# HandH1998/QQQ

Hardware: AMD Instinct MI355X
Metric: W4A8 GEMM TOPS + speedup vs fp16, M in {1..4096} N=8192 K=21760 (higher is better)
Workload: dtype i8 x i4 -> i32 -> f16; 1 GPU; qqq_gemm per-channel sweep M in {1,16,128,1024,4096} N=8192 K=21760 (configs[1]); step = the 5 calls; weights=12 rotating 89 MB int4 buffers (cold Infinity Cache), GPTQ-style N(0,0.02^2), launch=hipGraph replay, 1-step opener then 10 steps/graph, parallelism=single GPU

## Files before the change

qqq_amd/csrc/qqq_wide.hip.h:

```cpp
#ifndef QQQ_AMD_QQQ_WIDE_HIP_H_
#define QQQ_AMD_QQQ_WIDE_HIP_H_


#ifndef QQQ_WIDE_ABLATE
#define QQQ_WIDE_ABLATE 0
#endif
#ifdef QQQ_PANEL_TRACE
#define QQQ_WTRV(i, v)                                                                                   \
  do {                                                                                                   \
    if (wn == 0 && qqq_trace_buf) qqq_trace_buf[(size_t)blockIdx.x * 16 + (i)] = (unsigned long long)(v); \
  } while (0)
#define QQQ_WTR(i) QQQ_WTRV(i, wall_clock64())
#else
#define QQQ_WTR(i) do {} while (0)
#define QQQ_WTRV(i, v) do {} while (0)
#endif
template <int... S, class F>
__device__ __forceinline__ void qqq_static_for(std::integer_sequence<int, S...>, F&& f) {
  (f(std::integral_constant<int, S>{}), ...);
}
template <int N, class F>
__device__ __forceinline__ void qqq_static_for(F&& f) {
  qqq_static_for(std::make_integer_sequence<int, N>{}, static_cast<F&&>(f));
}

__device__ __forceinline__ __amdgpu_buffer_rsrc_t wide_view(const void* base_uniform) {
  return __builtin_amdgcn_make_buffer_rsrc(const_cast<void*>(base_uniform), 0, 0xffffffff, 0x00020000);
}
__device__ __forceinline__ v4u wide_load16(__amdgpu_buffer_rsrc_t view, const unsigned voff, const unsigned soff) {
  return __builtin_amdgcn_raw_buffer_load_b128(view, voff, soff, 0);
}

__host__ __device__ constexpr bool wide_frag_slot(int hw, int k) { return k % (2 * hw) == 2 * hw - 1; }
__host__ __device__ constexpr int wide_dw_load_index(int mt, int hw, int k) {
  if (hw == 2) {
    if (mt == 8) {
      constexpr int at[8] = {2, 5, 6, 10, 14, 18, 22, 26};
      for (int i = 0; i < 8; ++i)
        if (at[i] == k) return i;
      return -1;
    }
    return (k % 4 == 2 && k <= 30) ? (k - 2) / 4 : -1;
  }
  return k == 2 ? 0 : k == 8 ? 1 : k == 10 ? 2 : k == 16 ? 3 : -1;
}
__host__ __device__ constexpr int wide_ring_load(int mode, int mt, int hw, int k) {
  if (mode == 2) return k % ((2 * hw * mt) / (2 * hw)) == 2 ? k / ((2 * hw * mt) / (2 * hw)) : -1;
  return wide_dw_load_index(mt, hw, k);
}
__host__ __device__ constexpr int wide_ring_last_slot(int mt, int hw, int hf) {
  int last = 0;
  for (int k = 0; k < 2 * hw * mt; ++k)
    if (wide_dw_load_index(mt, hw, k) == 4 * hf + 3) last = k;
  return last;
}
__host__ __device__ constexpr int wide_dma_period(int mt, int hw) { return (2 * hw * mt) / (mt / 4); }
__host__ __device__ constexpr bool wide_m0_slot(int mt, int hw, int k) { return k % wide_dma_period(mt, hw) == (hw == 2 ? 8 : 4); }
__host__ __device__ constexpr bool wide_dma_slot(int mt, int hw, int k) { return k % wide_dma_period(mt, hw) == (hw == 2 ? 9 : 6); }
__host__ __device__ constexpr int wide_scale_slot(int hw) { return hw == 2 ? 1 : 0; }

__host__ __device__ constexpr int wide_w8_refill_index_(int mt, int hw, int k) { return k % ((2 * hw * mt) / (2 * hw)) == 2 ? k / ((2 * hw * mt) / (2 * hw)) : -1; }
__host__ __device__ constexpr bool wide_plain_slot(int mode, int mt, int hw, int k) {
  if (k < 0 || k >= 2 * hw * mt) return false;
  if (wide_frag_slot(hw, k) || wide_dma_slot(mt, hw, k) || wide_m0_slot(mt, hw, k)) return false;
  if (wide_ring_load(mode, mt, hw, k) >= 0) return false;
  if (mode == 1 && k == wide_scale_slot(hw)) return false;
  return true;
}
__host__ __device__ constexpr int wide_barrier_slot(int mode, int mt, int hw) {
  for (int k = 2 * hw * mt - 1; k >= 0; --k)
    if (wide_plain_slot(mode, mt, hw, k)) return k;
  return 0;
}
__host__ __device__ constexpr int wide_plain_after(int mode, int mt, int hw, int k0, int skip) {
  int last = -1;
  for (int k = k0 + 1; k < 2 * hw * mt; ++k)
    if (wide_plain_slot(mode, mt, hw, k) && k != wide_barrier_slot(mode, mt, hw)) {
      last = k;
      if (skip-- == 0) return k;
    }
  return last;
}
__host__ __device__ constexpr int wide_ring_inc_slot(int mode, int mt, int hw) {
  int last = 0;
  for (int k = 0; k < 2 * hw * mt; ++k)
    if (wide_ring_load(mode, mt, hw, k) >= 0) last = k;
  return wide_plain_after(mode, mt, hw, last, 1);
}
__host__ __device__ constexpr int wide_dma_inc_slot(int, int, int) { return 0; }
__host__ __device__ constexpr int wide_scale_inc_slot(int mode, int mt, int hw) { return wide_plain_after(mode, mt, hw, wide_scale_slot(hw), 2); }
__host__ __device__ constexpr int wide_bal_cap(int mode, int mt, int hw, int t, int k, int cursors) {
  if (!wide_plain_slot(mode, mt, hw, k)) return wide_m0_slot(mt, hw, k) && !wide_frag_slot(hw, k) && !wide_dma_slot(mt, hw, k) ? 1 : 0;
  int c = 2;
  if (t == 1 && k == wide_barrier_slot(mode, mt, hw)) c -= 2;
  if (cursors == 1) {
    if (k == wide_ring_inc_slot(mode, mt, hw)) c -= 1;
    if (t == 0 && k == wide_dma_inc_slot(mode, mt, hw)) c -= 1;
    if (mode == 1 && t == 1 && k == wide_scale_inc_slot(mode, mt, hw)) c -= 1;
  }
  return c < 0 ? 0 : c;
}
__host__ __device__ constexpr int wide_bal_items(int mode) { return 1 + (mode == 1 ? 32 : 12); }
__host__ __device__ constexpr int wide_bal_cost(int mode, int w) { return w == 0 ? 1 : (mode == 1 ? 2 : 1); }
__host__ __device__ constexpr int wide_bal_before(int mode, int mt, int hw, int t, int k, int cursors) {
  const int nslot = 2 * hw * mt, per = wide_bal_items(mode), ni = hw * per;
  int ct = 0, cb = 0, tc = 0;
  for (int j = 0; j < nslot; ++j) ct += wide_bal_cap(mode, mt, hw, t, j, cursors);
  for (int j = 0; j < k; ++j) cb += wide_bal_cap(mode, mt, hw, t, j, cursors);
  for (int i = 0; i < ni; ++i) tc += wide_bal_cost(mode, i % per);
  if (k >= nslot) return ni;
  int n = 0, e = 0;
  for (int i = 0; i < ni; ++i) {
    e += wide_bal_cost(mode, i % per);
    if ((long long)e * ct <= (long long)cb * tc) ++n;
  }
  return n;
}

template <int MODE, int MT, int HW, int T, int CURSORS>
struct WideBalTable {
  struct Tab {
    int before[2 * HW * MT + 1];
  };
  static constexpr Tab make() {
    Tab r{};
    constexpr int nslot = 2 * HW * MT, per = wide_bal_items(MODE), ni = HW * per;
    int cap[nslot] = {};
    int ct = 0, tc = 0;
    for (int j = 0; j < nslot; ++j) {
      cap[j] = wide_bal_cap(MODE, MT, HW, T, j, CURSORS);
      ct += cap[j];
    }
    for (int i = 0; i < ni; ++i) tc += wide_bal_cost(MODE, i % per);
    int cb = 0, n = 0, e = wide_bal_cost(MODE, 0);
    for (int k = 0; k < nslot; ++k) {
      while (n < ni && (long long)e * ct <= (long long)cb * tc) {
        ++n;
        if (n < ni) e += wide_bal_cost(MODE, n % per);
      }
      r.before[k] = n;
      cb += cap[k];
    }
    r.before[nslot] = ni;
    return r;
  }
  static constexpr Tab tab = make();
};

static_assert(WideBalTable<0, 16, 2, 0, 1>::tab.before[17] == wide_bal_before(0, 16, 2, 0, 17, 1) && WideBalTable<0, 16, 2, 1, 1>::tab.before[63] == wide_bal_before(0, 16, 2, 1, 63, 1) &&
                  WideBalTable<1, 8, 2, 1, 0>::tab.before[9] == wide_bal_before(1, 8, 2, 1, 9, 0) && WideBalTable<1, 16, 1, 0, 0>::tab.before[30] == wide_bal_before(1, 16, 1, 0, 30, 0),
              "the table is the function");

__host__ __device__ constexpr int wide_w8_refill_index(int mt, int hw, int k) {
  const int per = (2 * hw * mt) / (2 * hw);
  return k % per == 2 ? k / per : -1;
}
__host__ __device__ constexpr int wide_loads_in_slot(int mode, int mt, int hw, int t, int k) {
  int n = 0;
  if (mode == 1 && t == 1 && k == wide_scale_slot(hw) && !(QQQ_WIDE_ABLATE & 8)) n += 2;
  if (mode != 2 && wide_ring_load(mode, mt, hw, k) >= 0 && !(QQQ_WIDE_ABLATE & 8)) n += 1;
  if (mode == 2 && wide_w8_refill_index(mt, hw, k) >= 0 && !(QQQ_WIDE_ABLATE & 8)) n += 1;
  if (wide_dma_slot(mt, hw, k) && !(QQQ_WIDE_ABLATE & 2)) n += 1;
  return n;
}
__host__ __device__ constexpr int wide_loads_in_step(int mode, int mt, int hw, int t, int from, int to) {
  int n = 0;
  for (int k = from; k < to && k < 2 * hw * mt; ++k) n += wide_loads_in_slot(mode, mt, hw, t, k);
  return n;
}
__host__ __device__ constexpr int wide_loads_between(int mode, int mt, int hw, int t0, int k0, int steps, int k1) {
  int n = wide_loads_in_step(mode, mt, hw, t0, k0 + 1, 2 * hw * mt);
  for (int j = 1; j < steps; ++j) n += wide_loads_in_step(mode, mt, hw, (t0 + j) & 1, 0, 2 * hw * mt);
  return n + wide_loads_in_step(mode, mt, hw, (t0 + steps) & 1, 0, k1);
}
__host__ __device__ constexpr int wide_w8_last_refill_slot(int mt, int hw) {
  int last = 0;
  for (int k = 0; k < 2 * hw * mt; ++k) last = wide_w8_refill_index(mt, hw, k) >= 0 ? k : last;
  return last;
}
__host__ __device__ constexpr int wide_last_dma_slot(int mt, int hw) {
  int last = 0;
  for (int k = 0; k < 2 * hw * mt; ++k) last = wide_dma_slot(mt, hw, k) ? k : last;
  return last;
}

template <int MODE, int MT, int P, int RS, int HW, bool CHAIN = false>
__global__ __launch_bounds__(256) __attribute__((amdgpu_waves_per_eu(1, 1))) void qqq_wide_kernel(
    const int8_t* __restrict__ A, const unsigned char* __restrict__ B, int32_t* __restrict__ C, _Float16* __restrict__ D,
    const float* __restrict__ s1, const float* __restrict__ s2, const _Float16* __restrict__ s3,
    int32_t* __restrict__ acc_out, int* __restrict__ tickets, const _Float16* __restrict__ bias, const int M, const int N,
    const int K, const int tiles_m, const int tiles_n, const int PW, const int ksplit_hf) {
  const int ksplit = ksplit_hf & 0xffff, hflags = (ksplit_hf >> 16) & 0xff, skew = (ksplit_hf >> 24) & 0x3f;
  constexpr bool GROUPED = MODE == 1, W8 = MODE == 2;
  static_assert(MODE >= 0 && MODE <= 2, "0 per-channel, 1 per-group, 2 expanded int8");
  static_assert(!W8 || RS >= 3, "W8: a slot is refilled one step after its use -- RS - 1 steps of lead, the wait count needs at least one whole step in between");
  constexpr int RL = W8 ? RS - 1 : RS;
  static_assert(MT == 16 || MT == 8, "m-tiles of 16 tokens per wave (= per workgroup): 256 or 128 tokens");
  static_assert(HW == 2 || HW == 1, "a wave owns both 32-column halves of a 64-column group, or (128-column tiles) one");
  constexpr int ROWS = 16 * MT;
  constexpr int NQ = 2 * HW;
  constexpr int BN = 128 * HW;
  constexpr int NT = 256;
  constexpr int XB = ROWS * 128;
  constexpr int XPT = XB / 16 / NT;
  static_assert((2 * P) % RS == 0, "weight ring (in 64-k steps) must divide the unroll period");
  static_assert(P >= 4 && P <= 6, "LDS stage buffers: one being read, one complete, P - 2 in flight");
  constexpr int LA = P - 1;
  constexpr int NSLOT = NQ * MT;
  constexpr int EPR = HW == 2 ? 8 * MT : 16 * MT;
  constexpr int EP_STRIDE = BN + 4;

  extern __shared__ __attribute__((aligned(16))) unsigned char smem[];

  const int tid = threadIdx.x;
  const int lane = tid & 63;
  const int wn = __builtin_amdgcn_readfirstlane(tid >> 6);
  QQQ_WTR(0);

  int tile_m, tile_n, tile_lin, sp;
  auto locate = [&](const int lin, int& tm, int& tn) {
    const int full = (tiles_n / PW) * PW * tiles_m;
    if (lin < full) {
      const int panel = lin / (PW * tiles_m), within = lin % (PW * tiles_m);
      tm = within / PW;
      tn = panel * PW + within % PW;
    } else {
      const int rem = lin - full, pw = tiles_n % PW;
      tm = rem / pw;
      tn = (tiles_n / PW) * PW + rem % pw;
    }
  };
  int ch_first = 0, ch_stride = 0, ch_tiles = 1;
  {
    const int ntot = tiles_m * tiles_n * (CHAIN ? 1 : ksplit);
    const int bid = blockIdx.x;
    const int q = ntot >> 3, rr = ntot & 7;
    const int xcd = bid & 7, idx = bid >> 3;
    const int lin2 = (xcd < rr ? xcd * (q + 1) : rr * (q + 1) + (xcd - rr) * q) + idx;
    if constexpr (CHAIN) {
      const int cnt = q + (xcd < rr ? 1 : 0);
      ch_stride = (int)(gridDim.x >> 3);
      ch_first = lin2;
      ch_tiles = idx < cnt ? (cnt - idx + ch_stride - 1) / ch_stride : 0;
      if (ch_tiles == 0) return;
      sp = 0;
      tile_lin = lin2;
      locate(lin2, tile_m, tile_n);
    } else if (ksplit == 2 && (hflags & 16) != 0 && ((tiles_m * tiles_n) & 3) == 0) {
      const int per = (tiles_m * tiles_n) >> 2;
      sp = xcd & 1;
      tile_lin = (xcd >> 1) * per + idx;
      locate(tile_lin, tile_m, tile_n);
    } else {
      const int lin = lin2 / ksplit;
      sp = lin2 - lin * ksplit;
      tile_lin = lin;
      locate(lin, tile_m, tile_n);
    }
  }
  unsigned my_xcc = 0;
  if (!CHAIN && ksplit > 1) {
    asm volatile("s_getreg_b32 %0, hwreg(HW_REG_XCC_ID)" : "=s"(my_xcc));
    my_xcc &= 7u;
    if (tid == 0 && ksplit <= 6)
      __hip_atomic_fetch_or(tickets + 2 * (size_t)tile_lin, (int)((8u | my_xcc) << (8 + 4 * sp)), __ATOMIC_RELAXED, __HIP_MEMORY_SCOPE_AGENT);
  }
  const int mbase = tile_m * ROWS;
  const int ngroups = N >> 6;
  const int cb = tile_n * 4 + wn;
  int ng = HW == 2 ? cb : cb >> 1;
  const int whalf = HW == 2 ? 0 : (cb & 1);
  if (ng >= ngroups) ng = ngroups - 1;
  const unsigned rowbytes = (unsigned)N * 8u;
  const unsigned wstep = W8 ? (unsigned)N * 64u : 4u * rowbytes;

  const int NSE = (K >> 7) - skew;
  const int st0 = (int)(((long long)NSE * sp) / ksplit);
  const int NST = (sp == ksplit - 1 ? (K >> 7) : (int)(((long long)NSE * (sp + 1)) / ksplit)) - st0;
  const int KS = 2 * NST;

  const int h = lane >> 4, cq = (lane >> 2) & 3, q4 = lane & 3;
  auto descriptor = [](const void* base_uniform) {
    const unsigned long long a = (unsigned long long)base_uniform;
    return (v4u){(unsigned)__builtin_amdgcn_readfirstlane((int)a), (unsigned)__builtin_amdgcn_readfirstlane((int)(a >> 32)), 0xffffffffu,
                 0x00020000u};
  };
  v4u wdesc = descriptor(CHAIN ? (const void*)B : (const void*)(B + (size_t)ng * (W8 ? 4096 : 512)));
  constexpr bool CUR = !CHAIN;
  if constexpr (CUR) {
    const unsigned long long total = W8 ? (unsigned long long)K * (unsigned)N : ((unsigned long long)K * (unsigned)N) >> 1;
    wdesc[2] = (unsigned)__builtin_amdgcn_readfirstlane((int)(unsigned)(total - (unsigned long long)ng * (W8 ? 4096u : 512u)));
  }
  const unsigned woff = W8 ? (unsigned)(lane * 16 + 2048 * whalf)
                           : (unsigned)h * rowbytes + (unsigned)(cq * 64 + q4 * 16 + 256 * whalf);
  v4u sdesc = descriptor(GROUPED ? (CHAIN ? (const void*)s3 : (const void*)(s3 + (size_t)ng * 64)) : (const void*)B);
  if constexpr (CUR && GROUPED) sdesc[2] = (unsigned)__builtin_amdgcn_readfirstlane((int)((unsigned)(K >> 7) * (unsigned)N * 2u - (unsigned)ng * 128u));
  const unsigned soff_l = (unsigned)((cq * 8 + 2 * q4) * 2 + 64 * whalf);
  v4u xdesc = descriptor(A + (size_t)mbase * K);
  if constexpr (CUR) {
    const unsigned long long rest = (unsigned long long)(M - mbase) * (unsigned)K;
    xdesc[2] = (unsigned)__builtin_amdgcn_readfirstlane((int)(unsigned)(rest < 0xffffffffull ? rest : 0xffffffffull));
  }
  const int xr0 = tid >> 3, xslot = tid & 7;
  unsigned xoff[XPT];
#pragma unroll
  for (int q = 0; q < XPT; ++q) {
    int row = xr0 + 32 * q;
    if (!CHAIN && mbase + row >= M) row = M - 1 - mbase;
    xoff[q] = (unsigned)row * (unsigned)K + (unsigned)((xslot ^ ((xr0 >> 1) & 7)) * 16);
  }
  const unsigned lds_wave = (unsigned)wn * 1024u;

  auto tile_ref = [&](const int tm, const int tn, unsigned& a_lo, unsigned& a_hi, unsigned& a_rec, unsigned& w_so, unsigned& s_so) {
    const unsigned long long a = (unsigned long long)(A + (size_t)tm * ROWS * (size_t)K);
    a_lo = (unsigned)__builtin_amdgcn_readfirstlane((int)a);
    a_hi = (unsigned)__builtin_amdgcn_readfirstlane((int)(a >> 32));
    const int rows = M - tm * ROWS < ROWS ? M - tm * ROWS : ROWS;
    a_rec = (unsigned)__builtin_amdgcn_readfirstlane(rows * K);
    const int cbw = tn * 4 + wn;
    int g = HW == 2 ? cbw : cbw >> 1;
    if (g >= ngroups) g = ngroups - 1;
    w_so = (unsigned)__builtin_amdgcn_readfirstlane(g * (W8 ? 4096 : 512));
    s_so = (unsigned)__builtin_amdgcn_readfirstlane(g * 128);
  };
  int cur_tm = tile_m, cur_tn = tile_n, nx_tm = tile_m, nx_tn = tile_n, ch_pos = 0;
  unsigned cu_a_lo = 0, cu_a_hi = 0, cu_a_rec = 0, cu_w_so = 0, cu_s_so = 0;
  unsigned nx_a_lo = 0, nx_a_hi = 0, nx_a_rec = 0, nx_w_so = 0, nx_s_so = 0;
  unsigned cx_so = 0, cr_so = 0, cc_so = 0;
  auto sgpr = [](const unsigned v) { return (unsigned)__builtin_amdgcn_readfirstlane((int)v); };
  auto cursors_at_stage0 = [&]() {
    cx_so = (unsigned)LA * 128u;
    cr_so = sgpr(cu_w_so + (unsigned)RL * wstep);
    cc_so = sgpr(cu_s_so + (unsigned)P * (unsigned)N * 2u);
    xdesc[0] = sgpr(cu_a_lo), xdesc[1] = sgpr(cu_a_hi), xdesc[2] = sgpr(cu_a_rec);
  };
  if constexpr (CHAIN) {
    tile_ref(tile_m, tile_n, cu_a_lo, cu_a_hi, cu_a_rec, cu_w_so, cu_s_so);
    if (ch_tiles > 1) locate(ch_first + ch_stride, nx_tm, nx_tn);
    tile_ref(nx_tm, nx_tn, nx_a_lo, nx_a_hi, nx_a_rec, nx_w_so, nx_s_so);
    cursors_at_stage0();
  }

  auto dma_m0 = [&](auto bufc, auto qc) __attribute__((always_inline)) {
    constexpr unsigned dst = (unsigned)(decltype(bufc)::value * XB + decltype(qc)::value * 4096);
    (void)lds_wave;
    asm volatile("s_add_u32 m0, %0, %1" : : "s"(lds_wave), "n"(dst) : "scc");
  };
  auto dma_go = [&](auto qc, unsigned so) __attribute__((always_inline)) {
    (void)xoff[0], (void)xdesc;
    so = __builtin_amdgcn_readfirstlane(so);
    asm("" : "+s"(so));
    asm volatile("buffer_load_dwordx4 %0, %1, %2 offen lds" : : "v"(xoff[decltype(qc)::value]), "s"(xdesc), "s"(so) : "memory");
  };
  auto dma_go_cur = [&](auto qc) __attribute__((always_inline)) {
    (void)xoff[0], (void)xdesc, (void)cx_so;
    asm volatile("buffer_load_dwordx4 %0, %1, %2 offen lds" : : "v"(xoff[decltype(qc)::value]), "s"(xdesc), "s"(cx_so) : "memory");
  };
  auto dma_x = [&](auto bufc, auto qc, const unsigned so) __attribute__((always_inline)) {
    dma_m0(bufc, qc);
    asm volatile("s_nop 0");
    dma_go(qc, so);
  };
  auto dma_stage_so = [&](auto bufc, const unsigned so) __attribute__((always_inline)) {
    qqq_static_for<XPT>([&](auto qc) { dma_x(bufc, qc, so); });
  };
  auto dma_stage = [&](auto bufc, const int st_rel) __attribute__((always_inline)) {
    const int st = st_rel < NST ? st_rel : NST - 1;
    dma_stage_so(bufc, (unsigned)(st0 + st) * 128u);
  };
  auto asm_load_w = [&](v4u& dst, auto hfc, unsigned so) __attribute__((always_inline)) {
    (void)woff, (void)wdesc;
    so = __builtin_amdgcn_readfirstlane(so);
    asm("" : "+s"(so));
    if constexpr ((QQQ_W_NT & 8) != 0)
      asm volatile("buffer_load_dwordx4 %0, %1, %2, %3 offen offset:%4 nt" : "=v"(dst) : "v"(woff), "s"(wdesc), "s"(so), "n"((W8 ? 1024 : 256) * decltype(hfc)::value));
    else
      asm volatile("buffer_load_dwordx4 %0, %1, %2, %3 offen offset:%4" : "=v"(dst) : "v"(woff), "s"(wdesc), "s"(so), "n"((W8 ? 1024 : 256) * decltype(hfc)::value));
  };
  auto asm_load_w_cur = [&](v4u& dst, auto hfc) __attribute__((always_inline)) {
    (void)woff, (void)wdesc, (void)cr_so;
    asm volatile("buffer_load_dwordx4 %0, %1, %2, %3 offen offset:%4" : "=v"(dst) : "v"(woff), "s"(wdesc), "s"(cr_so), "n"((W8 ? 1024 : 256) * decltype(hfc)::value));
  };
  constexpr int WRN = W8 ? NQ : HW;
  auto load_w_so = [&](const unsigned so, v4u (&dst)[WRN]) __attribute__((always_inline)) {
    qqq_static_for<WRN>([&](auto hfc) { asm_load_w(dst[decltype(hfc)::value], hfc, so); });
  };
  auto load_w = [&](const int step_rel, v4u (&dst)[WRN]) __attribute__((always_inline)) {
    const int s = step_rel < KS ? step_rel : KS - 1;
    load_w_so((unsigned)(2 * st0 + s) * wstep, dst);
  };
  auto load_sc_so = [&](unsigned so, unsigned (&dst)[2]) __attribute__((always_inline)) {
    so = __builtin_amdgcn_readfirstlane(so);
    asm("" : "+s"(so));
    asm volatile("buffer_load_dword %0, %1, %2, %3 offen" : "=v"(dst[0]) : "v"(soff_l), "s"(sdesc), "s"(so));
    asm volatile("buffer_load_dword %0, %1, %2, %3 offen offset:%4" : "=v"(dst[1]) : "v"(soff_l), "s"(sdesc), "s"(so), "n"(HW == 2 ? 64 : 0));
  };
  auto load_sc_cur = [&](unsigned (&dst)[2]) __attribute__((always_inline)) {
    (void)cc_so;
    asm volatile("buffer_load_dword %0, %1, %2, %3 offen" : "=v"(dst[0]) : "v"(soff_l), "s"(sdesc), "s"(cc_so));
    asm volatile("buffer_load_dword %0, %1, %2, %3 offen offset:%4" : "=v"(dst[1]) : "v"(soff_l), "s"(sdesc), "s"(cc_so), "n"(HW == 2 ? 64 : 0));
  };
  auto load_sc = [&](const int st_rel, unsigned (&dst)[2]) __attribute__((always_inline)) {
    const int st = st_rel < NST ? st_rel : NST - 1;
    load_sc_so((unsigned)(st0 + st) * (unsigned)N * 2u, dst);
  };

  v4i acc[MT][NQ];
#pragma unroll
  for (int mt = 0; mt < MT; ++mt)
#pragma unroll
    for (int q = 0; q < NQ; ++q) acc[mt][q] = (v4i){0, 0, 0, 0};

  v4u wr[RS][WRN];
  constexpr bool DW = !W8;
  unsigned wq[DW ? RS : 1][HW][4];
  const unsigned woff_dw = (unsigned)h * rowbytes + (unsigned)(cq * 64 + q4 * 4 + 256 * whalf);
  auto asm_load_d = [&](unsigned& dst, auto ic, unsigned so, auto rawc) __attribute__((always_inline)) {
    constexpr int li = decltype(ic)::value;
    (void)woff_dw, (void)wdesc;
    if constexpr (!decltype(rawc)::value) {
      so = __builtin_amdgcn_readfirstlane(so);
      asm("" : "+s"(so));
    }
    asm volatile("buffer_load_dword %0, %1, %2, %3 offen offset:%4" : "=v"(dst) : "v"(woff_dw), "s"(wdesc), "s"(so), "n"(256 * (li / 4) + 16 * (li % 4)));
  };
  auto load_d_step = [&](const unsigned so, unsigned (&dst)[HW][4]) __attribute__((always_inline)) {
    qqq_static_for<4 * HW>([&](auto ic) { asm_load_d(dst[decltype(ic)::value / 4][decltype(ic)::value % 4], ic, so, std::false_type{}); });
  };
  unsigned scr[GROUPED ? P : 1][2];
  v4i x[MT];
  v4i aop[2][NQ];
  const unsigned xrd = (unsigned)((lane & 15) * 128);
  const int xsw = ((lane & 15) >> 1) & 7;
  const unsigned xrd_t[2] = {xrd + (unsigned)(((0 + h) ^ xsw) << 4), xrd + (unsigned)(((4 + h) ^ xsw) << 4)};

  auto read_x = [&](const int buf, const int t, const int mt) {
    x[mt] = *reinterpret_cast<const v4i*>(smem + buf * XB + xrd_t[t] + mt * 2048);
  };

  const unsigned nmask = QQQ_NIB_MASK;
  h2 sb[2];
  unsigned gt0[2] = {0, 0}, gt1[2] = {0, 0};
  h2 gha[2], ghb[2];
  constexpr int UPARTS = GROUPED ? 32 : 12;
  auto un_setup = [&](const h2 sc) {
    if constexpr (GROUPED) {
      sb[0] = (h2){sc[0], sc[0]};
      sb[1] = (h2){sc[1], sc[1]};
    }
  };
  auto un_part = [&](auto pc, auto hfc, v4i (&a)[NQ], const unsigned (&y)[4]) {
    constexpr int pi = decltype(pc)::value, hf = decltype(hfc)::value;
    if constexpr (GROUPED) {
      constexpr int kq = pi / 8, part = (pi % 8) / 2, b = pi % 2;
      if constexpr (part == 0) {
        const unsigned qv = b ? (y[kq] >> 8) : y[kq];
        const unsigned magic = qqq_fp16_1024x2();
        gt0[b] = (qv & 0x000f000fu) | magic;
        gt1[b] = (qv & 0x00f000f0u) | magic;
      } else if constexpr (part == 1) {
        const h2 c_sub = {(_Float16)-1032.0f, (_Float16)-1032.0f};
        const h2 c_mul = {(_Float16)0.0625f, (_Float16)0.0625f};
        const h2 c_add = {(_Float16)-72.0f, (_Float16)-72.0f};
        gha[b] = __builtin_bit_cast(h2, gt0[b]) + c_sub;
        ghb[b] = __builtin_elementwise_fma(__builtin_bit_cast(h2, gt1[b]), c_mul, c_add);
      } else if constexpr (part == 2) {
        const h2 c_mag = {(_Float16)1152.0f, (_Float16)1152.0f};
        gha[b] = __builtin_elementwise_fma(gha[b], sb[b], c_mag);
        ghb[b] = __builtin_elementwise_fma(ghb[b], sb[b], c_mag);
      } else {
        int w = (int)(__builtin_amdgcn_perm(__builtin_bit_cast(unsigned, ghb[b]), __builtin_bit_cast(unsigned, gha[b]), 0x06040200u) ^ 0x80808080u);
        if constexpr (CHAIN) asm volatile("" : "+v"(w));
        a[2 * hf + b][kq] = w;
      }
    } else {
      constexpr int kq = pi / 3, part = pi % 3;
      if constexpr (part == 0) {
        int w = (int)(y[kq] & nmask);
        asm volatile("" : : "v"(w));
        a[2 * hf][kq] = w;
      } else if constexpr (part == 1) {
        gt0[0] = y[kq] << 4;
        asm volatile("" : : "v"(gt0[0]));
      } else {
        int w = (int)(gt0[0] & nmask);
        asm volatile("" : : "v"(w));
        a[2 * hf + 1][kq] = w;
      }
    }
  };
  auto mfma = [&](v4i& c, const auto& wa, const v4i& xb) {
    asm volatile("v_mfma_i32_16x16x64_i8 %0, %1, %2, %0" : "+a"(c) : "v"(wa), "v"(xb));
  };

  unsigned st_xso = 0, st_swo[2] = {0, 0}, st_sco = 0;
  auto step = [&](const int i, auto uc, auto tc) __attribute__((always_inline)) {
    constexpr int t = decltype(tc)::value, u = decltype(uc)::value;
    constexpr int cur = t, nxt = 1 - t;
    constexpr int sl = (2 * u + t) % RS, sn = (sl + 1) % RS;
    constexpr int su = GROUPED ? ((t == 1) ? (u + 1) % P : u) : 0;
    const unsigned cswo = st_swo[t], csco = st_sco;
    constexpr int BSLOT = wide_barrier_slot(MODE, MT, HW);
    static_assert(!CUR || (wide_ring_inc_slot(MODE, MT, HW) > 0 && (!GROUPED || wide_scale_inc_slot(MODE, MT, HW) > wide_scale_slot(HW))), "every cursor has a slot behind its last use");
    auto slot = [&](auto kc) __attribute__((always_inline)) {
      constexpr int k = decltype(kc)::value, mt = k / NQ, q = k % NQ;
      if constexpr (W8) mfma(acc[mt][q], wr[sl][q], x[mt]);
      else mfma(acc[mt][q], aop[cur][q], x[mt]);
      __builtin_amdgcn_sched_barrier(0);
      if constexpr (W8) {
        if constexpr (k == NSLOT - 1) {
          constexpr int younger_all = wide_loads_between(MODE, MT, HW, 0, wide_w8_last_refill_slot(MT, HW), RL - 1, NSLOT);
          constexpr int younger = younger_all < 63 ? younger_all : 63;
          if constexpr (HW == 2) asm volatile("s_waitcnt vmcnt(%4)" : "+v"(wr[sn][0]), "+v"(wr[sn][1]), "+v"(wr[sn][2]), "+v"(wr[sn][3]) : "n"(younger));
          else asm volatile("s_waitcnt vmcnt(%2)" : "+v"(wr[sn][0]), "+v"(wr[sn][1]) : "n"(younger));
        }
      } else if constexpr (!(QQQ_WIDE_ABLATE & 4)) {
        constexpr int PER = wide_bal_items(MODE);
        constexpr int FIX = CUR ? 1 : 0;
        constexpr int lo = WideBalTable<MODE, MT, HW, t, FIX>::tab.before[k], hi = WideBalTable<MODE, MT, HW, t, FIX>::tab.before[k + 1];
        qqq_static_for<(hi - lo)>([&](auto jc) {
          constexpr int it = lo + decltype(jc)::value;
          constexpr int hf = it / PER, w_ = it % PER;
          if constexpr (w_ == 0) {
            constexpr int younger_all = wide_loads_between(MODE, MT, HW, (t + RS - 1) & 1, wide_ring_last_slot(MT, HW, hf), RS - 1, k);
            constexpr int younger = younger_all < 63 ? younger_all : 63;
            (void)wq[0][0][0];
            if constexpr (GROUPED && CHAIN && HW == 1) asm volatile("s_waitcnt vmcnt(%6)" : "+v"(wq[sn][hf][0]), "+v"(wq[sn][hf][1]), "+v"(wq[sn][hf][2]), "+v"(wq[sn][hf][3]), "+v"(scr[su][0]), "+v"(scr[su][1]) : "n"(younger));
            else if constexpr (GROUPED) asm volatile("s_waitcnt vmcnt(%5)" : "+v"(wq[sn][hf][0]), "+v"(wq[sn][hf][1]), "+v"(wq[sn][hf][2]), "+v"(wq[sn][hf][3]), "+v"(scr[su][hf]) : "n"(younger));
            else asm volatile("s_waitcnt vmcnt(%4)" : "+v"(wq[sn][hf][0]), "+v"(wq[sn][hf][1]), "+v"(wq[sn][hf][2]), "+v"(wq[sn][hf][3]) : "n"(younger));
            un_setup(__builtin_bit_cast(h2, scr[su][hf]));
          } else {
            un_part(std::integral_constant<int, w_ - 1>{}, std::integral_constant<int, hf>{}, aop[nxt], wq[sn][hf]);
          }
        });
      } else if constexpr (k == 0) {
        qqq_static_for<NQ>([&](auto qc) {
          constexpr int qq = decltype(qc)::value;
          aop[nxt][qq] = (v4i){(int)wr[sn][qq / 2][0], (int)wr[sn][qq / 2][1], (int)wr[sn][qq / 2][2], (int)wr[sn][qq / 2][3]};
        });
      }
      if constexpr (wide_frag_slot(HW, k) && !(QQQ_WIDE_ABLATE & 16)) {
        read_x(t == 0 ? (u % P) : ((u + 1) % P), t == 0 ? 1 : 0, mt);
// ... 32 lines not shown
        }
      }
      constexpr int DP = wide_dma_period(MT, HW);
      if constexpr (wide_m0_slot(MT, HW, k) && !(QQQ_WIDE_ABLATE & 2))
        dma_m0(std::integral_constant<int, (u + LA) % P>{}, std::integral_constant<int, (XPT / 2) * t + k / DP>{});
      if constexpr (wide_dma_slot(MT, HW, k) && !(QQQ_WIDE_ABLATE & 2)) {
        if constexpr (CUR) dma_go_cur(std::integral_constant<int, (XPT / 2) * t + k / DP>{});
        else dma_go(std::integral_constant<int, (XPT / 2) * t + k / DP>{}, st_xso);
      }
      if constexpr (t == 1 && k == BSLOT) {
        constexpr int since = wide_loads_between(MODE, MT, HW, 1, wide_last_dma_slot(MT, HW), 2 * (P - 3), k + 1);
        static_assert(since < 64, "vmcnt is a 6-bit counter");
        if constexpr (!(QQQ_WIDE_ABLATE & 1)) asm volatile("s_waitcnt vmcnt(%0)\n\ts_barrier" : : "n"(since) : "memory");
        else asm volatile("s_waitcnt vmcnt(%0)" : : "n"(since) : "memory");
      }
      __builtin_amdgcn_sched_barrier(0);
    };
    qqq_static_for<NSLOT>(slot);
  };

  constexpr int SCB = ROWS * 4 + BN * 6;
  constexpr int SC0 = P * XB;
  const int cej = lane & 15, cecp = lane >> 4;
  const int cegrp = HW == 2 ? wn : (wn >> 1), cehalf = wn & 1;
  auto scale_dma = [&](const int tm, const int tn, const int par) __attribute__((always_inline)) {
    const unsigned voff = (unsigned)((64 * wn + lane) * 4);
    const int rows = M - tm * ROWS < ROWS ? M - tm * ROWS : ROWS, cols = N - tn * BN < BN ? N - tn * BN : BN;
    auto one = [&](const void* base, const unsigned bytes, const unsigned dst) {
      v4u d = descriptor(base);
      d[2] = (unsigned)__builtin_amdgcn_readfirstlane((int)bytes);
      const unsigned m0v = (unsigned)__builtin_amdgcn_readfirstlane((int)dst);
      asm volatile("s_mov_b32 m0, %2\n\ts_nop 4\n\tbuffer_load_dword %0, %1, 0 offen lds" : : "v"(voff), "s"(d), "s"(m0v) : "memory");
    };
    const unsigned r0 = (unsigned)(SC0 + par * SCB + 256 * wn);
    if (wn < ROWS / 64) one(s1 + (size_t)tm * ROWS, (unsigned)rows * 4u, r0);
    if (wn < BN / 64) one(s2 + (size_t)tn * BN, (unsigned)cols * 4u, r0 + ROWS * 4);
    if (wn < BN / 128 && bias) one(bias + (size_t)tn * BN, (unsigned)cols * 2u, r0 + ROWS * 4 + BN * 4);
  };
  auto flush_tile = [&](const int tm, const int tn, const int par) __attribute__((always_inline)) {
    asm volatile("s_nop 15\n\ts_nop 15" ::: "memory");
    const unsigned char* sc = smem + SC0 + par * SCB;
    const float* s1t = reinterpret_cast<const float*>(sc);
    const float* s2t = reinterpret_cast<const float*>(sc + ROWS * 4);
    const _Float16* bt = reinterpret_cast<const _Float16*>(sc + ROWS * 4 + BN * 4);
    const _Float16 nzc = (_Float16)-0.0f;
    const int cl = 64 * cegrp + 16 * cecp;
    const bool cols_ok = tn * BN + 64 * cegrp < N;
    float2 dsa[NQ], dsb[NQ];
    h4 dbv[NQ];
    int dl[NQ];
#pragma unroll
    for (int q = 0; q < NQ; ++q) {
      dl[q] = cl + 8 * (q & 1) + 4 * (HW == 2 ? (q >> 1) : cehalf);
      const int i0 = s2_stored_index(dl[q]);
      dsa[q] = *reinterpret_cast<const float2*>(s2t + i0);
      dsb[q] = *reinterpret_cast<const float2*>(s2t + i0 + 8);
      dbv[q] = (h4){nzc, nzc, nzc, nzc};
    }
    if (bias) {
#pragma unroll
      for (int q = 0; q < NQ; ++q) dbv[q] = *reinterpret_cast<const h4*>(bt + dl[q]);
    }
    v4i zero4 = {0, 0, 0, 0};
    asm volatile("" : "+v"(zero4));
    const int rows = M - tm * ROWS < ROWS ? M - tm * ROWS : ROWS;
    const __amdgpu_buffer_rsrc_t dview = __builtin_amdgcn_make_buffer_rsrc(D + (size_t)tm * ROWS * N, 0, rows * N * 2, 0x00020000);
    const __amdgpu_buffer_rsrc_t aview = __builtin_amdgcn_make_buffer_rsrc(acc_out ? acc_out + (size_t)tm * ROWS * N : (int32_t*)D, 0, rows * N * 4, 0x00020000);
    const unsigned drow = (unsigned)(cej * N + tn * BN) * 2u;
#pragma unroll
    for (int mt = 0; mt < MT; ++mt) {
      const float ts = s1t[16 * mt + cej];
      h4 o[NQ];
#pragma unroll
      for (int q = 0; q < NQ; q += 2) {
        v4i ra = acc[mt][q], rb = acc[mt][q + 1];
        asm volatile("" : "+v"(ra), "+v"(rb));
        asm volatile("v_mfma_i32_16x16x64_i8 %0, %1, %1, 0" : "+a"(acc[mt][q]) : "v"(zero4));
        asm volatile("v_mfma_i32_16x16x64_i8 %0, %1, %1, 0" : "+a"(acc[mt][q + 1]) : "v"(zero4));
        int a0 = ra[0], a1 = ra[1], a2 = ra[2], a3 = ra[3], b0 = rb[0], b1 = rb[1], b2 = rb[2], b3 = rb[3];
        asm volatile("s_nop 1\n\t"
                     "v_permlane16_swap_b32 %0, %1\n\tv_permlane16_swap_b32 %2, %3\n\t"
                     "v_permlane16_swap_b32 %4, %5\n\tv_permlane16_swap_b32 %6, %7\n\t"
                     "v_permlane32_swap_b32 %0, %2\n\tv_permlane32_swap_b32 %1, %3\n\t"
                     "v_permlane32_swap_b32 %4, %6\n\tv_permlane32_swap_b32 %5, %7"
                     : "+v"(a0), "+v"(a1), "+v"(a2), "+v"(a3), "+v"(b0), "+v"(b1), "+v"(b2), "+v"(b3));
        if (acc_out && cols_ok) {
          const unsigned ar = (drow + (unsigned)(16 * mt) * (unsigned)N * 2u) * 2u;
          __builtin_amdgcn_raw_buffer_store_b128((v4u){(unsigned)a0, (unsigned)a1, (unsigned)a2, (unsigned)a3}, aview, ar + (unsigned)dl[q] * 4u, 0, 0);
          __builtin_amdgcn_raw_buffer_store_b128((v4u){(unsigned)b0, (unsigned)b1, (unsigned)b2, (unsigned)b3}, aview, ar + (unsigned)dl[q + 1] * 4u, 0, 0);
        }
        o[q] = epilogue_vals4(a0, a1, a2, a3, ts, dsa[q], dsb[q]) + dbv[q];
        o[q + 1] = epilogue_vals4(b0, b1, b2, b3, ts, dsa[q + 1], dsb[q + 1]) + dbv[q + 1];
      }
      if (cols_ok) {
        const unsigned dr = drow + (unsigned)(16 * mt) * (unsigned)N * 2u;
        if constexpr (HW == 2) {
          const h8 lo8 = {o[0][0], o[0][1], o[0][2], o[0][3], o[2][0], o[2][1], o[2][2], o[2][3]};
          const h8 hi8 = {o[1][0], o[1][1], o[1][2], o[1][3], o[3][0], o[3][1], o[3][2], o[3][3]};
          __builtin_amdgcn_raw_buffer_store_b128(__builtin_bit_cast(v4u, lo8), dview, dr + (unsigned)cl * 2u, 0, 0);
          __builtin_amdgcn_raw_buffer_store_b128(__builtin_bit_cast(v4u, hi8), dview, dr + (unsigned)cl * 2u + 16u, 0, 0);
        } else {
          typedef unsigned v2u __attribute__((ext_vector_type(2)));
#pragma unroll
          for (int q = 0; q < NQ; ++q) __builtin_amdgcn_raw_buffer_store_b64(__builtin_bit_cast(v2u, o[q]), dview, dr + (unsigned)dl[q] * 2u, 0, 0);
        }
      }
      __builtin_amdgcn_sched_barrier(0);
    }
  };
  auto seam = [&]() __attribute__((always_inline)) {
    QQQ_WTRV(ch_pos < 7 ? 2 + 2 * ch_pos : 15, wall_clock64());
    flush_tile(cur_tm, cur_tn, ch_pos & 1);
    QQQ_WTRV(ch_pos < 7 ? 3 + 2 * ch_pos : 15, wall_clock64());
    ++ch_pos;
    cur_tm = nx_tm, cur_tn = nx_tn;
    cu_a_lo = nx_a_lo, cu_a_hi = nx_a_hi, cu_a_rec = nx_a_rec, cu_w_so = nx_w_so, cu_s_so = nx_s_so;
    if (ch_pos < ch_tiles) {
      scale_dma(cur_tm, cur_tn, ch_pos & 1);
      if (ch_pos + 1 < ch_tiles) locate(ch_first + (ch_pos + 1) * ch_stride, nx_tm, nx_tn);
      nx_tm = __builtin_amdgcn_readfirstlane(nx_tm), nx_tn = __builtin_amdgcn_readfirstlane(nx_tn);
      tile_ref(nx_tm, nx_tn, nx_a_lo, nx_a_hi, nx_a_rec, nx_w_so, nx_s_so);
    }
    cursors_at_stage0();
  };

  constexpr int RST = NT / (BN / 8);
  const int c8 = tid % (BN / 8), er0 = tid / (BN / 8);
  const int n = tile_n * BN + c8 * 8;
  float2 s2v[4] = {};
  const _Float16 nz = (_Float16)-0.0f;
  h8 bv = {nz, nz, nz, nz, nz, nz, nz, nz};
  if (!CHAIN && n < N) {
    const int i0s = s2_stored_index(n), i1s = s2_stored_index(n + 4);
    s2v[0] = *reinterpret_cast<const float2*>(s2 + i0s);
    s2v[1] = *reinterpret_cast<const float2*>(s2 + i0s + 8);
    s2v[2] = *reinterpret_cast<const float2*>(s2 + i1s);
    s2v[3] = *reinterpret_cast<const float2*>(s2 + i1s + 8);
    if (bias) bv = *reinterpret_cast<const h8*>(bias + n);
  }

  if constexpr (CHAIN) {
    scale_dma(tile_m, tile_n, 0);
    qqq_static_for<LA>([&](auto jc) { dma_stage_so(jc, (unsigned)decltype(jc)::value * 128u); });
#pragma unroll
    for (int j = 0; j < RL; ++j) {
      if constexpr (DW) load_d_step(cu_w_so + (unsigned)j * wstep, wq[j]);
      else load_w_so(cu_w_so + (unsigned)j * wstep, wr[j]);
    }
    if constexpr (GROUPED) {
#pragma unroll
      for (int j = 0; j < P; ++j) load_sc_so(cu_s_so + (unsigned)j * (unsigned)N * 2u, scr[j]);
    }
  } else {
    qqq_static_for<LA>([&](auto jc) { dma_stage(jc, decltype(jc)::value); });
#pragma unroll
    for (int j = 0; j < RL; ++j) {
      if constexpr (DW) load_d_step((unsigned)(2 * st0 + (j < KS ? j : KS - 1)) * wstep, wq[j]);
      else load_w(j, wr[j]);
    }
    if constexpr (GROUPED) {
#pragma unroll
      for (int j = 0; j < P; ++j) load_sc(j, scr[j]);
    }
  }
  qqq_static_for<RL>([&](auto jc) {
    constexpr int j = decltype(jc)::value;
    (void)wr[0];
    if constexpr (DW) {
      (void)wq[0][0][0];
      qqq_static_for<HW>([&](auto hfc) {
        constexpr int hf = decltype(hfc)::value;
        (void)wq[0][0][0];
        asm volatile("s_waitcnt vmcnt(0)" : "+v"(wq[j][hf][0]), "+v"(wq[j][hf][1]), "+v"(wq[j][hf][2]), "+v"(wq[j][hf][3]));
      });
    } else if constexpr (HW == 2) asm volatile("s_waitcnt vmcnt(0)" : "+v"(wr[j][0]), "+v"(wr[j][1]), "+v"(wr[j][2]), "+v"(wr[j][3]));
    else asm volatile("s_waitcnt vmcnt(0)" : "+v"(wr[j][0]), "+v"(wr[j][1]));
  });
  if constexpr (GROUPED) {
    qqq_static_for<P>([&](auto jc) {
      (void)scr[0];
      asm volatile("" : "+v"(scr[decltype(jc)::value][0]), "+v"(scr[decltype(jc)::value][1]));
    });
  }
  __syncthreads();
#pragma unroll
  for (int mt = 0; mt < MT; ++mt) read_x(0, 0, mt);
  if constexpr (!W8) {
    qqq_static_for<HW>([&](auto hfc) {
      constexpr int hf = decltype(hfc)::value;
      un_setup(__builtin_bit_cast(h2, scr[0][hf]));
      (void)wq[0][0][0];
      qqq_static_for<UPARTS>([&](auto pc) { un_part(pc, hfc, aop[0], wq[0][hf]); });
    });
  }
  __builtin_amdgcn_sched_barrier(0);

  if constexpr (CUR) {
    cx_so = sgpr((unsigned)(st0 + LA - 1) * 128u);
    cr_so = sgpr((unsigned)(2 * st0 + RL) * wstep);
    cc_so = sgpr((unsigned)(st0 + P) * (unsigned)N * 2u);
  }
  auto do_stage = [&](const int i, auto uc) __attribute__((always_inline)) {
    step(i, uc, std::integral_constant<int, 0>{});
    step(i, uc, std::integral_constant<int, 1>{});
  };
  QQQ_WTR(1);
  if constexpr (CHAIN) {
    static_assert(!CHAIN || P == 4, "the trip is written out for four stage buffers");
    int left = NST;
    auto do_stage_chain = [&](auto uc) __attribute__((always_inline)) {
      const unsigned sstep = (unsigned)N * 2u;
      if (__builtin_expect(left > P, 1)) {
        st_xso = sgpr(cx_so), st_swo[0] = sgpr(cr_so), st_swo[1] = sgpr(cr_so + wstep), st_sco = sgpr(cc_so);
        cx_so += 128u, cr_so += 2u * wstep, cc_so += sstep;
        asm volatile("" : "+s"(st_xso), "+s"(st_swo[0]), "+s"(st_swo[1]), "+s"(st_sco));
      } else {
        const int done = NST - left;
        const bool xn = left <= LA, cn = true;
        st_xso = sgpr(xn ? (unsigned)(LA - left) * 128u : (unsigned)(done + LA) * 128u);
        xdesc[0] = sgpr(xn ? nx_a_lo : cu_a_lo), xdesc[1] = sgpr(xn ? nx_a_hi : cu_a_hi), xdesc[2] = sgpr(xn ? nx_a_rec : cu_a_rec);
#pragma unroll
        for (int t = 0; t < 2; ++t) {
          const int sn_ = 2 * done + t + RL;
          st_swo[t] = sgpr(sn_ < KS ? cu_w_so + (unsigned)sn_ * wstep : nx_w_so + (unsigned)(sn_ - KS) * wstep);
        }
        st_sco = sgpr(cn ? nx_s_so + (unsigned)(P - left) * sstep : 0u);
        asm volatile("s_nop 4" : "+s"(st_xso), "+s"(st_swo[0]), "+s"(st_swo[1]), "+s"(st_sco), "+s"(xdesc));
      }
      step(0, uc, std::integral_constant<int, 0>{});
      step(0, uc, std::integral_constant<int, 1>{});
    };
    bool more = true;
#define QQQ_CHAIN_STAGE(U)                                    \
  if (__builtin_expect(more, 1)) {                            \
    do_stage_chain(std::integral_constant<int, U>{});         \
    if (__builtin_expect(--left == 0, 0)) {                   \
      seam();                                                 \
      left = NST;                                             \
      if (ch_pos == ch_tiles) {                               \
        asm volatile("s_waitcnt vmcnt(0)" ::: "memory");      \
        more = false;                                         \
      }                                                       \
    }                                                         \
  }
    do {
      QQQ_CHAIN_STAGE(0)
      QQQ_CHAIN_STAGE(1)
      QQQ_CHAIN_STAGE(2)
      QQQ_CHAIN_STAGE(3)
    } while (more);
    return;
#undef QQQ_CHAIN_STAGE
  }
  int i0 = 0;
  for (; i0 + P <= NST; i0 += P) {
#if defined(QQQ_PANEL_TRACE) && defined(QQQ_WIDE_TRACE_TRIPS)
    if (i0 < 12 * P) QQQ_WTRV(4 + i0 / P, __builtin_amdgcn_s_memtime());
#endif
    qqq_static_for<P>([&](auto uc) __attribute__((always_inline)) { do_stage(i0 + decltype(uc)::value, uc); });
  }
  qqq_static_for<P - 1>([&](auto uc) __attribute__((always_inline)) {
    if (i0 + decltype(uc)::value < NST) do_stage(i0 + decltype(uc)::value, uc);
  });

  asm volatile("s_waitcnt vmcnt(0)" ::: "memory");
  if constexpr (DW) {
    qqq_static_for<RS * HW>([&](auto jc) {
      constexpr int j = decltype(jc)::value / HW, hf = decltype(jc)::value % HW;
      (void)wq[0][0][0];
      asm volatile("" : : "v"(wq[j][hf][0]), "v"(wq[j][hf][1]), "v"(wq[j][hf][2]), "v"(wq[j][hf][3]));
    });
  }
  qqq_static_for<RS>([&](auto jc) {
    (void)wr[0];
    if constexpr (DW) return;
    asm volatile("" : : "v"(wr[decltype(jc)::value][0]), "v"(wr[decltype(jc)::value][WRN - 1]));
    if constexpr (W8 && HW == 2) asm volatile("" : : "v"(wr[decltype(jc)::value][1]), "v"(wr[decltype(jc)::value][2]));
  });
  if constexpr (GROUPED) {
    qqq_static_for<P>([&](auto jc) {
      (void)scr[0];
      asm volatile("" : : "v"(scr[decltype(jc)::value][0]), "v"(scr[decltype(jc)::value][1]));
    });
  }
  QQQ_WTR(2);
  asm volatile("s_nop 15\n\ts_nop 15" ::: "memory");
  int* ep = reinterpret_cast<int*>(smem);
  const int ej = lane & 15, ecp = lane >> 4;
  const int egrp = HW == 2 ? wn : (wn >> 1), ehalf = wn & 1;
  constexpr int EP_ITEMS = EPR * (BN / 8), EP_PASSES = EP_ITEMS / NT;
  auto image = [&](const int pass) __attribute__((always_inline)) {
#pragma unroll
    for (int jm = 0; jm < EPR / 16; ++jm)
#pragma unroll
      for (int q = 0; q < NQ; ++q)
#pragma unroll
        for (int r = 0; r < 4; ++r)
          ep[(16 * jm + ej) * EP_STRIDE + 64 * egrp + 16 * r + 8 * (q & 1) + 4 * (HW == 2 ? (q >> 1) : ehalf) + ecp] = acc[pass * (EPR / 16) + jm][q][r];
  };

  constexpr unsigned XB_EXCH = 1u << 16, XB_CLASSIC = 1u << 17;
  const bool exch_on = ksplit == 2 && (hflags & 8) != 0 && ROWS / EPR == 2;
  int arrival = 0;
  bool exch = false;
  if (ksplit > 1) {
    int* tk = tickets + 2 * (size_t)tile_lin;
    int* xch = ep + EPR * EP_STRIDE;
    if (tid == 0) {
      unsigned w = (unsigned)__hip_atomic_fetch_add(tk, 1, __ATOMIC_RELAXED, __HIP_MEMORY_SCOPE_AGENT);
      if (exch_on) {
        const unsigned arr = w & 0xffu;
        if (arr == 0) {
          const unsigned dec = (((w >> (8 + 4 * (1 - sp))) & 8u) != 0) ? XB_EXCH : XB_CLASSIC;
          (void)__hip_atomic_fetch_or(tk, (int)dec, __ATOMIC_RELAXED, __HIP_MEMORY_SCOPE_AGENT);
          w |= dec;
        } else {
          int spin = 0;
          while (!(w & (XB_EXCH | XB_CLASSIC))) {
            if (++spin > QQQ_SPIN_LIMIT) __builtin_trap();
            __builtin_amdgcn_s_sleep(1);
            w = (unsigned)__hip_atomic_load(tk, __ATOMIC_RELAXED, __HIP_MEMORY_SCOPE_AGENT);
          }
          w = (w & ~0xffu) | arr;
        }
      }
      *xch = (int)w;
    }
    __syncthreads();
    const unsigned word = (unsigned)__builtin_amdgcn_readfirstlane(*xch);
    arrival = (int)(word & 0xffu);
    exch = exch_on && (word & XB_EXCH) != 0;
#ifndef QQQ_WIDE_TRACE_TRIPS
    QQQ_WTR(4);
    QQQ_WTRV(7, (arrival << 1) | (exch ? 1 : 0));
#endif
    const size_t slot_ints = (size_t)ROWS * BN;
    if (exch || arrival < ksplit - 1) {
// ... 183 lines not shown
```

Baseline: 2893 TOPS.

## Replay steady-state load schedule in prologue and wait only on first stage

```diff
diff --git a/qqq_amd/csrc/qqq_wide.hip.h b/qqq_amd/csrc/qqq_wide.hip.h
--- a/qqq_amd/csrc/qqq_wide.hip.h
+++ b/qqq_amd/csrc/qqq_wide.hip.h
@@ -155,17 +155,18 @@
   const int per = (2 * hw * mt) / (2 * hw);
   return k % per == 2 ? k / per : -1;
 }
-__host__ __device__ constexpr int wide_loads_in_slot(int mode, int mt, int hw, int t, int k) {
+constexpr int WIDE_LD_DMA = 1, WIDE_LD_RING = 2, WIDE_LD_SCALE = 4, WIDE_LD_ALL = 7;
+__host__ __device__ constexpr int wide_loads_in_slot(int mode, int mt, int hw, int t, int k, int kinds = WIDE_LD_ALL) {
   int n = 0;
-  if (mode == 1 && t == 1 && k == wide_scale_slot(hw) && !(QQQ_WIDE_ABLATE & 8)) n += 2;
-  if (mode != 2 && wide_ring_load(mode, mt, hw, k) >= 0 && !(QQQ_WIDE_ABLATE & 8)) n += 1;
-  if (mode == 2 && wide_w8_refill_index(mt, hw, k) >= 0 && !(QQQ_WIDE_ABLATE & 8)) n += 1;
-  if (wide_dma_slot(mt, hw, k) && !(QQQ_WIDE_ABLATE & 2)) n += 1;
+  if ((kinds & WIDE_LD_SCALE) && mode == 1 && t == 1 && k == wide_scale_slot(hw) && !(QQQ_WIDE_ABLATE & 8)) n += 2;
+  if ((kinds & WIDE_LD_RING) && mode != 2 && wide_ring_load(mode, mt, hw, k) >= 0 && !(QQQ_WIDE_ABLATE & 8)) n += 1;
+  if ((kinds & WIDE_LD_RING) && mode == 2 && wide_w8_refill_index(mt, hw, k) >= 0 && !(QQQ_WIDE_ABLATE & 8)) n += 1;
+  if ((kinds & WIDE_LD_DMA) && wide_dma_slot(mt, hw, k) && !(QQQ_WIDE_ABLATE & 2)) n += 1;
   return n;
 }
-__host__ __device__ constexpr int wide_loads_in_step(int mode, int mt, int hw, int t, int from, int to) {
+__host__ __device__ constexpr int wide_loads_in_step(int mode, int mt, int hw, int t, int from, int to, int kinds = WIDE_LD_ALL) {
   int n = 0;
-  for (int k = from; k < to && k < 2 * hw * mt; ++k) n += wide_loads_in_slot(mode, mt, hw, t, k);
+  for (int k = from; k < to && k < 2 * hw * mt; ++k) n += wide_loads_in_slot(mode, mt, hw, t, k, kinds);
   return n;
 }
 __host__ __device__ constexpr int wide_loads_between(int mode, int mt, int hw, int t0, int k0, int steps, int k1) {
@@ -182,6 +183,22 @@
   int last = 0;
   for (int k = 0; k < 2 * hw * mt; ++k) last = wide_dma_slot(mt, hw, k) ? k : last;
   return last;
+}
+__host__ __device__ constexpr int wide_fill_kinds(int s, int la, int rl) {
+  return (s >= -2 * la ? WIDE_LD_DMA : 0) | (s >= -rl ? WIDE_LD_RING : 0) | WIDE_LD_SCALE;
+}
+__host__ __device__ constexpr int wide_fill_younger(int mode, int mt, int hw, int la, int rl, int s0, int k0) {
+  int n = wide_loads_in_step(mode, mt, hw, s0 & 1, k0 + 1, 2 * hw * mt, wide_fill_kinds(s0, la, rl));
+  for (int s = s0 + 1; s < 0; ++s) n += wide_loads_in_step(mode, mt, hw, s & 1, 0, 2 * hw * mt, wide_fill_kinds(s, la, rl));
+  return n;
+}
+__host__ __device__ constexpr int wide_fill_wait(int mode, int mt, int hw, int la, int rl) {
+  int ring_last = 0;
+  for (int k = 0; k < 2 * hw * mt; ++k)
+    if ((mode == 2 ? wide_w8_refill_index(mt, hw, k) : wide_dw_load_index(mt, hw, k)) >= 0) ring_last = k;
+  const int a = wide_fill_younger(mode, mt, hw, la, rl, 2 * (1 - la) + 1, wide_last_dma_slot(mt, hw));
+  const int b = wide_fill_younger(mode, mt, hw, la, rl, -rl, ring_last);
+  return a < b ? a : b;
 }
 
 template <int MODE, int MT, int P, int RS, int HW, bool CHAIN = false>
@@ -364,10 +381,6 @@
   auto dma_stage_so = [&](auto bufc, const unsigned so) __attribute__((always_inline)) {
     qqq_static_for<XPT>([&](auto qc) { dma_x(bufc, qc, so); });
   };
-  auto dma_stage = [&](auto bufc, const int st_rel) __attribute__((always_inline)) {
-    const int st = st_rel < NST ? st_rel : NST - 1;
-    dma_stage_so(bufc, (unsigned)(st0 + st) * 128u);
-  };
   auto asm_load_w = [&](v4u& dst, auto hfc, unsigned so) __attribute__((always_inline)) {
     (void)woff, (void)wdesc;
     so = __builtin_amdgcn_readfirstlane(so);
@@ -384,10 +397,6 @@
   constexpr int WRN = W8 ? NQ : HW;
   auto load_w_so = [&](const unsigned so, v4u (&dst)[WRN]) __attribute__((always_inline)) {
     qqq_static_for<WRN>([&](auto hfc) { asm_load_w(dst[decltype(hfc)::value], hfc, so); });
-  };
-  auto load_w = [&](const int step_rel, v4u (&dst)[WRN]) __attribute__((always_inline)) {
-    const int s = step_rel < KS ? step_rel : KS - 1;
-    load_w_so((unsigned)(2 * st0 + s) * wstep, dst);
   };
   auto load_sc_so = [&](unsigned so, unsigned (&dst)[2]) __attribute__((always_inline)) {
     so = __builtin_amdgcn_readfirstlane(so);
@@ -726,18 +735,56 @@
       for (int j = 0; j < P; ++j) load_sc_so(cu_s_so + (unsigned)j * (unsigned)N * 2u, scr[j]);
     }
   } else {
-    qqq_static_for<LA>([&](auto jc) { dma_stage(jc, decltype(jc)::value); });
-#pragma unroll
-    for (int j = 0; j < RL; ++j) {
-      if constexpr (DW) load_d_step((unsigned)(2 * st0 + (j < KS ? j : KS - 1)) * wstep, wq[j]);
-      else load_w(j, wr[j]);
-    }
+    static_assert(2 * P >= RL && 2 * P >= 2 * LA, "the fill replays 2 P steps");
+    qqq_static_for<2 * P>([&](auto jc) {
+      constexpr int s = decltype(jc)::value - 2 * P, t = s & 1, i = (s - t) / 2, u = ((i % P) + P) % P;
+      constexpr int kinds = wide_fill_kinds(s, LA, RL);
+      constexpr int DP = wide_dma_period(MT, HW);
+      const int fs = s + RL < KS ? s + RL : KS - 1, fx = i + LA < NST ? i + LA : NST - 1;
+      const unsigned fso = (unsigned)(2 * st0 + fs) * wstep, fxo = (unsigned)(st0 + fx) * 128u;
+      (void)fso, (void)fxo;
+      qqq_static_for<NSLOT>([&](auto kc) {
+        constexpr int k = decltype(kc)::value;
+        if constexpr (GROUPED && (kinds & WIDE_LD_SCALE) != 0 && t == 1 && k == wide_scale_slot(HW)) load_sc(i + P, scr[u]);
+        if constexpr ((kinds & WIDE_LD_RING) != 0) {
+          constexpr int sl = (s + RL) % RS;
+          if constexpr (W8) {
+            constexpr int j = wide_w8_refill_index(MT, HW, k);
+            if constexpr (j >= 0) asm_load_w(wr[sl][j], std::integral_constant<int, j>{}, fso);
+          } else {
+            constexpr int li = wide_dw_load_index(MT, HW, k);
+            if constexpr (li >= 0) asm_load_d(wq[sl][li / 4][li % 4], std::integral_constant<int, li>{}, fso, std::false_type{});
+          }
+        }
+        if constexpr ((kinds & WIDE_LD_DMA) != 0 && wide_dma_slot(MT, HW, k))
+          dma_x(std::integral_constant<int, (u + LA) % P>{}, std::integral_constant<int, (XPT / 2) * t + k / DP>{}, fxo);
+      });
+    });
+  }
+  if constexpr (!CHAIN) {
+    constexpr int FW = wide_fill_wait(MODE, MT, HW, LA, RL);
+    static_assert(FW >= 0 && FW < 64, "vmcnt is a 6-bit counter");
+#pragma unroll
+    for (int mt = 0; mt < MT; ++mt)
+#pragma unroll
+      for (int q = 0; q < NQ; ++q) asm volatile("" : "+a"(acc[mt][q]));
+    (void)wr[0];
+    if constexpr (DW) {
+      (void)wq[0][0][0];
+      qqq_static_for<HW>([&](auto hfc) {
+        constexpr int hf = decltype(hfc)::value;
+        (void)wq[0][0][0];
+        asm volatile("s_waitcnt vmcnt(%4)" : "+v"(wq[0][hf][0]), "+v"(wq[0][hf][1]), "+v"(wq[0][hf][2]), "+v"(wq[0][hf][3]) : "n"(FW));
+      });
+    } else if constexpr (HW == 2) asm volatile("s_waitcnt vmcnt(%4)" : "+v"(wr[0][0]), "+v"(wr[0][1]), "+v"(wr[0][2]), "+v"(wr[0][3]) : "n"(FW));
+    else asm volatile("s_waitcnt vmcnt(%2)" : "+v"(wr[0][0]), "+v"(wr[0][1]) : "n"(FW));
     if constexpr (GROUPED) {
-#pragma unroll
-      for (int j = 0; j < P; ++j) load_sc(j, scr[j]);
-    }
-  }
-  qqq_static_for<RL>([&](auto jc) {
+      (void)scr[0];
+      asm volatile("" : "+v"(scr[0][0]), "+v"(scr[0][1]));
+    }
+    asm volatile("s_barrier" ::: "memory");
+  }
+  qqq_static_for<(CHAIN ? RL : 0)>([&](auto jc) {
     constexpr int j = decltype(jc)::value;
     (void)wr[0];
     if constexpr (DW) {
@@ -750,13 +797,13 @@
     } else if constexpr (HW == 2) asm volatile("s_waitcnt vmcnt(0)" : "+v"(wr[j][0]), "+v"(wr[j][1]), "+v"(wr[j][2]), "+v"(wr[j][3]));
     else asm volatile("s_waitcnt vmcnt(0)" : "+v"(wr[j][0]), "+v"(wr[j][1]));
   });
-  if constexpr (GROUPED) {
+  if constexpr (CHAIN && GROUPED) {
     qqq_static_for<P>([&](auto jc) {
       (void)scr[0];
       asm volatile("" : "+v"(scr[decltype(jc)::value][0]), "+v"(scr[decltype(jc)::value][1]));
     });
   }
-  __syncthreads();
+  if constexpr (CHAIN) __syncthreads();
 #pragma unroll
   for (int mt = 0; mt < MT; ++mt) read_x(0, 0, mt);
   if constexpr (!W8) {
```

Result: no change. 2902 TOPS, median of 4 (+0.3%).
